# RikVoorhaar/tt-sketch

Hardware: AMD Instinct MI355X
Metric: TT-cores sketched/sec (fp64) + achieved MFMA % for d=6 n=200 r=50 stream_sketch (higher is better)
Workload: dtype f64

## Files before the change

### include/ttsk.h

```cpp
#ifndef TTSK_H
#define TTSK_H

#include <stddef.h>
#include <stdint.h>

#ifdef __cplusplus
extern "C" {
#endif

typedef enum {
    TTSK_OK = 0,
    TTSK_ERR_HIP = -1,
    TTSK_ERR_ARG = -2,
    TTSK_ERR_UNSUPPORTED = -3,
    TTSK_ERR_COMM = -4
} ttsk_status;

#define TTSK_NUM_STREAMS 8

int ttsk_init(int device);
int ttsk_shutdown(void);
const char *ttsk_last_error(void);
int ttsk_device_info(char *name, size_t name_len, int *num_cu, size_t *hbm_bytes);
int ttsk_malloc(void **dev, size_t bytes);
// ... 38 lines not shown
                         double *out, int64_t out_stride, int accumulate, int stream);
int ttsk_tt_sketch_sum(int nb, int d, const int64_t *n, const int64_t *s, const int64_t *lt, const int64_t *l_lo,
                       const int64_t *l_hi, const int64_t *rt, const int64_t *r_lo, const int64_t *r_hi,
                       const double *const *X, const double *const *DL, const double *const *DR,
                       double *out, int accumulate, int stream);
int ttsk_chain_step(int nb, int n, int K1, int A, int A2, int J, const double *const *W, int64_t w_c,
                    const double *const *X, int64_t x_j, int64_t x_k, int64_t x_c, int64_t x_extent,
                    const double *E, double *const *T, double *const *Out, int stream);
int ttsk_chain_step_wide(int nb, int n, int K1, int A, int A2, int J, const double *const *W, int64_t w_c,
                         const double *const *X, int64_t x_j, int64_t x_k, int64_t x_c, int64_t x_extent,
                         const double *E, double *const *T, double *const *Out, int stream);
int ttsk_chain_step_sum(int nb, int n, int K1, int A, int A2, int J, const double *const *W, int64_t w_c,
                        const double *const *X, int64_t x_j, int64_t x_k, int64_t x_c, int64_t x_extent,
                        const double *E, double *T, int64_t t_b, int64_t t_ld, int64_t t_extent,
                        double *const *Out, int stream);
int ttsk_dense_left_pass(const double *X, int64_t n0, int64_t n1, int64_t n2, int64_t C, int64_t n4, int l,
                         const double *A0, const double *A1t, const double *A2t, const double *A3, double *Z0, double *Z1,
                         double *Z2, double *E3, int stream);
int64_t ttsk_tt_sketch_size(int d, const int64_t *n, const int64_t *l_lo, const int64_t *l_hi,
                            const int64_t *r_lo, const int64_t *r_hi);
int ttsk_prof_enable(int on);
int ttsk_mfma_f64_peak_probe(double *tflops);
int ttsk_ndtri_rate_probe(double *gsamples);
int ttsk_prof_read(int cls, int64_t *launches, double *total_ms, double *flops);
int ttsk_prof_kernel_name(int cls, char *buf, size_t len);

int ttsk_hash_u64(uint64_t *host_vals, size_t n);
int ttsk_inds_to_rand_double(const uint64_t *host_idx, const uint64_t *shape, int m, size_t N,
                             int rank_min, int rank_max, uint64_t seed, double *host_out);
int ttsk_inds_to_normal(const int64_t *host_idx, const uint64_t *shape, int m, size_t N,
// ... 131 lines not shown
```

### tt_sketch_amd/_native.py

```python
import ctypes
import os
import re
from ctypes import POINTER, Structure, c_char_p, c_double, c_float, c_int, c_int64, c_size_t, c_uint64, c_void_p
from typing import NamedTuple, Optional

_HERE = os.path.dirname(os.path.abspath(__file__))
LIB_PATH = os.environ.get("TTSK_LIB") or os.path.join(_HERE, "libttsk.so")
HEADER_PATH = os.path.join(os.path.dirname(_HERE), "include", "ttsk.h")

TTSK_ERR_ARG = -2
TTSK_ERR_UNSUPPORTED = -3
NUM_STREAMS = 8


class TtskError(RuntimeError):
    """A HIP / RCCL level failure inside libttsk."""


class TtskUnsupported(TtskError):
    """The fused kernel does not cover this shape (caller composes from ttsk_gemm)."""


class GemmDesc(Structure):
    _fields_ = [(n, c_int64) for n in
# ... 46 lines not shown
    "ttsk_timer_stop": Entry([I, POINTER(c_float)]),
    "ttsk_graph_begin": Entry([I]),
    "ttsk_graph_end": Entry([I, POINTER(P)]),
    "ttsk_graph_launch": Entry([P, I], QUEUE),
    "ttsk_graph_free": Entry([P]),
    "ttsk_gemm": Entry([POINTER(GemmDesc), P, P, P, P, I], QUEUE),
    "ttsk_copy_strided": Entry([P, P, I, POINTER(I64), POINTER(I64), POINTER(I64), I], QUEUE),
    "ttsk_axpby": Entry([P, P, c_double, c_double, S, I], QUEUE),
    "ttsk_sum_slices": Entry([P, P, I, S, S, I, I], QUEUE),
    "ttsk_tt_sketch": Entry([I] + [POINTER(I64)] * 8 + [POINTER(P)] * 3 + [P, I, I], FORK_NEXT),
    "ttsk_tt_sketch_batch": Entry([I, I] + [POINTER(I64)] * 8 + [POINTER(P)] * 3 + [P, I64, I, I], FORK_NEXT),
    "ttsk_tt_sketch_sum": Entry([I, I] + [POINTER(I64)] * 8 + [POINTER(P)] * 3 + [P, I, I], FORK_NEXT),
    "ttsk_chain_step": Entry(_CHAIN + [POINTER(P), POINTER(P), I], QUEUE),
    "ttsk_chain_step_wide": Entry(_CHAIN + [POINTER(P), POINTER(P), I], QUEUE),
    "ttsk_chain_step_sum": Entry(_CHAIN + [P, I64, I64, I64, POINTER(P), I], QUEUE),
    "ttsk_dense_left_pass": Entry([P, I64, I64, I64, I64, I64, I, P, P, P, P, P, P, P, P, I], QUEUE),
    "ttsk_tt_sketch_size": Entry([I] + [POINTER(I64)] * 5, restype=I64),
    "ttsk_prof_enable": Entry([I]),
    "ttsk_mfma_f64_peak_probe": Entry([POINTER(c_double)]),
    "ttsk_ndtri_rate_probe": Entry([POINTER(c_double)]),
    "ttsk_prof_read": Entry([I, POINTER(I64), POINTER(c_double), POINTER(c_double)]),
    "ttsk_prof_kernel_name": Entry([I, c_char_p, S]),
    "ttsk_hash_u64": Entry([P, S]),
    "ttsk_inds_to_rand_double": Entry([P, P, I, S, I, I, U64, P]),
    "ttsk_inds_to_normal": Entry([P, P, I, S, I, I, U64, P]),
    "ttsk_inds_to_sparse_sign": Entry([P, P, I, S, I, I, I, I, U64, P]),
    "ttsk_sparse_normal_dev": Entry([P, I64, POINTER(I), POINTER(U64), I, S, I, I, U64, P, I], QUEUE),
    "ttsk_sparse_normal_table": Entry([POINTER(U64), I, I, I, U64, P, I], QUEUE),
    "ttsk_sparse_sign_dev": Entry([P, I64, POINTER(I), POINTER(U64), I, S, I, I, I, I, U64, P, I], QUEUE),
    "ttsk_sparse_sign_table": Entry([POINTER(U64), I, I, I, I, I, U64, P, I], QUEUE),
# ... 159 lines not shown
```

### tt_sketch_amd/csrc/chain_fused.h

```cpp
#pragma once
#include "chain_plan.h"
#include "skinny.h"

namespace ttsk {

#ifdef TTSK_LAB
#define CF_DIAG(bit) (a.diag & (bit))
#define CF_STAMP(i) do { if (a.stamps && blockIdx.x == 0 && lane == 0 && k - k_beg < 8) a.stamps[((k - k_beg) * CD_WAVES + w) * 8 + (i)] = __builtin_amdgcn_s_memtime(); } while (0)
#else
#define CF_DIAG(bit) 0
#define CF_STAMP(i) do { } while (0)
#endif
#define CF_BARRIER() do { if (!CF_DIAG(4)) lds_barrier(); } while (0)

template <int NQF, int STRQ, int NNF, int STRN, int D, bool WT, int EBUF, int UNR, int KIND, int APC = 0>
__device__ __forceinline__ void cf_piece(const ChainStep &a, const double *Wl, const double *El, int tile, int q0, int prob,
                                         int g, int k_beg, int k_end, int KB1, int w, int lane)
{
    const int x16 = lane & 15, kq = lane >> 4;
    const int AP = APC ? APC : a.AP, A2P = a.A2P;
    const int j0 = 16 * tile;
    const bool jok = j0 + x16 < a.J;
    const uint32_t xlane = !CF_DIAG(1) ? (uint32_t)(((int64_t)(j0 + x16) * a.x_j + (int64_t)kq * a.x_c) * 8) : OOB_OFF;
    const __amdgpu_buffer_rsrc_t rx = make_rsrc(uniform_ptr(a.X[prob]), a.x_extent * 8);
// ... 5 lines not shown
    double ring[D];
#pragma unroll
    for (int d = 0; d < D; ++d) ring[d] = xload((uint32_t)k_beg * kstep + (uint32_t)d * xstep);

    v4d acc2[NNF ? NNF : 1];
    double acc2s[STRN ? STRN : 1];
#pragma unroll
    for (int p = 0; p < NNF; ++p)
#pragma unroll
        for (int t = 0; t < 4; ++t) acc2[p][t] = 0.0;
#pragma unroll
    for (int q = 0; q < STRN; ++q) acc2s[q] = 0.0;

    const int wl_lane = (kq >> 1) * 2 * AP + 2 * (16 * q0 + x16) + (kq & 1);
    const int ws_lane = (kq >> 1) * 2 * AP + 2 * (16 * (q0 + NQF) + (x16 & 3)) + (kq & 1);
    const int el_lane = (kq >> 1) * 2 * A2P + 4 * (x16 >> 1) + 2 * (kq & 1) + (x16 & 1);
    const int es_col = 16 * NNF + (x16 & 3);
    const int es_lane = (kq >> 1) * 2 * A2P + 2 * (kq & 1);

    __amdgpu_buffer_rsrc_t rt;
    if constexpr (WT) rt = make_rsrc(uniform_ptr(a.T[prob]), a.t_extent * 8);

    for (int k = k_beg; k < k_end; ++k) {
        v4d acc1[NQF ? NQF : 1];
        double acc1s[STRQ ? STRQ : 1];
#pragma unroll
        for (int p = 0; p < NQF; ++p)
#pragma unroll
            for (int t = 0; t < 4; ++t) acc1[p][t] = 0.0;
#pragma unroll
        for (int q = 0; q < STRQ; ++q) acc1s[q] = 0.0;

        CF_STAMP(0);
// ... 37 lines not shown
            for (int p = 0; p < NQF; ++p)
#pragma unroll
                for (int t = 0; t < 4; ++t)
                    st8(rt, (jok && a0 + 16 * p + 4 * t + kq < a.A) ? tl + (uint32_t)((16 * p + 4 * t) * nJ * 8) : OOB_OFF, acc1[p][t]);
#pragma unroll
            for (int q = 0; q < STRQ; ++q)
                st8(rt, (jok && a0 + 16 * NQF + 4 * q + kq < a.A) ? tl + (uint32_t)((16 * NQF + 4 * q) * nJ * 8) : OOB_OFF, acc1s[q]);
        }
        CF_STAMP(1);
        CF_BARRIER();
        CF_STAMP(2);

        {
            const double *eb = El + (EBUF == 2 ? (k & 1) * a.eunits * 2 : 0) + q0 * 16 * A2P;
            double bf[NNF ? NNF : 1], bs[STRN ? STRN : 1];
            int el0 = el_lane, es0 = es_lane + 4 * (es_col >> 1) + (es_col & 1);
            asm volatile("" : "+v"(el0), "+v"(es0));
            auto efetch = [&](int kap, double (&f)[NNF ? NNF : 1], double (&g)[STRN ? STRN : 1]) {
#pragma unroll
                for (int nn = 0; nn < NNF; ++nn) f[nn] = LDS_UNPAIRED(eb[el0 + kap * 4 * A2P + 32 * nn]);
#pragma unroll
                for (int q = 0; q < STRN; ++q) g[q] = eb[es0 + kap * 4 * A2P + 8 * q];
            };
            double bf2[NNF ? NNF : 1], bs2[STRN ? STRN : 1];
            efetch(0, bf, bs);
            constexpr int KB2C = 4 * NQF + STRQ;
#pragma unroll
            for (int kap = 0; kap < KB2C; ++kap) {
                const int p = kap >> 2, t = kap & 3;
                const double af2 = p < NQF ? acc1[p < NQF ? p : 0][t] : acc1s[t < STRQ ? t : 0];
                if (kap & 1) {
// ... 62 lines not shown
    const __amdgpu_buffer_rsrc_t rx = make_rsrc(uniform_ptr(a.X[prob]), a.x_extent * 8);
    const uint32_t xstep = __builtin_amdgcn_readfirstlane((uint32_t)(4 * a.x_c * 8));
    const uint32_t kstep = __builtin_amdgcn_readfirstlane((uint32_t)(a.x_k * 8));
    const int ITER = KB1 / UNR;
    auto xload = [&](uint32_t so) -> double { return ld8(rx, xlane, __builtin_amdgcn_readfirstlane(so)); };
    double ring[D];
#pragma unroll
    for (int d = 0; d < D; ++d) ring[d] = xload((uint32_t)k_beg * kstep + (uint32_t)d * xstep);

    double acc2[NC];
#pragma unroll
    for (int c = 0; c < NC; ++c) acc2[c] = 0.0;

    const int wl_lane = (kq >> 1) * 2 * AP + 2 * x16 + (kq & 1);
    const int ws_lane = (kq >> 1) * 2 * AP + 2 * (16 * NQF + n4) + (kq & 1);
    const int el_lane = (2 * beta + (kq >> 1)) * 2 * A2P + 4 * (n4 >> 1) + 2 * (kq & 1) + (n4 & 1);
    const int es_lane = (kq >> 1) * 2 * A2P + 4 * (n4 >> 1) + 2 * (kq & 1) + (n4 & 1);

    __amdgpu_buffer_rsrc_t rt;
    if constexpr (WT) rt = make_rsrc(uniform_ptr(a.T[prob]), a.t_extent * 8);

    for (int k = k_beg; k < k_end; ++k) {
        double acc1[NQF], acc1s[STRQ ? STRQ : 1];
#pragma unroll
        for (int p = 0; p < NQF; ++p) acc1[p] = 0.0;
#pragma unroll
        for (int q = 0; q < STRQ; ++q) acc1s[q] = 0.0;
        CF_STAMP(0);
        uint32_t so = (uint32_t)k * kstep + (uint32_t)D * xstep;
        for (int it = 0; it < ITER; ++it) {
            const double *wrun = Wl + it * UNR * 4 * AP;
            const bool last = it == ITER - 1;
// ... 96 lines not shown
                const int c = e / AP, col = e - c * AP;
                if (e < total) Wl[(c >> 1) * 2 * AP + 2 * col + (c & 1)] = v[u];
            }
        }
    }

    unsigned pc = 0;
    int li = 0, nl = 1;
    if constexpr (NWV != 8) {
        pc = a.piece[__builtin_amdgcn_readfirstlane(w)];
        li = __builtin_amdgcn_readfirstlane((pc >> 8) & 255);
        nl = a.nload;
    }
    if (NWV == 8 ? w == 7 : __builtin_amdgcn_readfirstlane(pc >> 16) == CD_NONE) {
        if constexpr (NWV != 8) __builtin_amdgcn_s_setprio(3);
        const int NI = CF_DIAG(2) ? 0 : a.eunits >> 6;
        const uint32_t inv = (uint32_t)(((1ull << 32) + (uint32_t)A2P - 1) / (uint32_t)A2P);
        const int64_t rowstride = (int64_t)a.n * a.A2;
        const int ebuf = a.eunits * 2;
        auto fill = [&](int k) {
            const double *Ek = a.E + (int64_t)k * a.A2;
            double *dst = El + (EBUF == 2 ? (k & 1) * ebuf : 0);
#pragma unroll 2
            for (int m = li; m < NI; m += nl) {
                const uint32_t U = 64u * (uint32_t)m + (uint32_t)lane;
                const uint32_t sec = (uint32_t)(((uint64_t)U * inv) >> 32), u = U - sec * (uint32_t)A2P;
                int row = (int)(2 * sec + (u & 1));
                row = row < a.A ? row : a.A - 1;
                int col = (int)(2 * (u >> 1));
                col = col + 1 < a.A2 ? col : 0;
                __builtin_amdgcn_global_load_lds((const __attribute__((address_space(1))) void *)(Ek + row * rowstride + col),
                                                 (__attribute__((address_space(3))) void *)(dst + m * 128), 16, 0, 0);
            }
        };
        __syncthreads();
        if constexpr (EBUF == 2) {
            if (k_beg < k_end) fill(k_beg);
            for (int k = k_beg; k < k_end; ++k) {
                asm volatile("s_waitcnt vmcnt(0)" ::: "memory");
                CF_STAMP(1);
                CF_BARRIER();
                CF_STAMP(2);
                if (k + 1 < k_end) fill(k + 1);
                CF_STAMP(3);
                CF_BARRIER();
                CF_STAMP(4);
            }
        } else {
// ... 19 lines not shown
        const int kind = __builtin_amdgcn_readfirstlane(pc >> 16), tile = __builtin_amdgcn_readfirstlane(pc & 255);
        constexpr int H = cd_cut(NQF), APC = 16 * NQF + 4 * STRQ;
        if (kind == CD_WHOLE)
            cf_piece<NQF, STRQ, NNF, STRN, D, WT, EBUF, UNR, CD_WHOLE, APC>(a, Wl, El, tile, 0, prob, g, k_beg, k_end, KB1, w, lane);
        else if (kind == CD_FIRST)
            cf_piece<H, 0, NNF, STRN, D, WT, EBUF, UNR, CD_FIRST, APC>(a, Wl, El, tile, 0, prob, g, k_beg, k_end, KB1, w, lane);
        else if (kind == CD_REST)
            cf_piece<NQF - H, STRQ, NNF, STRN, D, WT, EBUF, UNR, CD_REST, APC>(a, Wl, El, tile, H, prob, g, k_beg, k_end, KB1, w, lane);
        else if (kind == CD_ROWS4)
            cf_rows4<NQF, STRQ, NNF, STRN, D, WT, EBUF, UNR, APC>(a, Wl, El, tile, prob, g, k_beg, k_end, KB1, w, lane);
    }
}

int chain_fused_try(const ChainStepArgs &c, int stream, hipStream_t st, bool force = false);

}
```

### tt_sketch_amd/csrc/chain_fused.hip

```cpp
#include <cstdlib>
#include "chain_fused.h"
#include "prof.h"

namespace ttsk {

int launch_chain_step_a(const ChainStep &a, int nf, int str, bool wt, int ebuf, int unr, int waves, size_t lds, int grid, hipStream_t st);
int launch_chain_step_b(const ChainStep &a, int nf, int str, bool wt, int ebuf, int unr, int waves, size_t lds, int grid, hipStream_t st);
int launch_chain_step_c(const ChainStep &a, int nf, int str, bool wt, int ebuf, int unr, int waves, size_t lds, int grid, hipStream_t st);
int launch_chain_step_d(const ChainStep &a, int nf, int str, bool wt, int ebuf, int unr, int waves, size_t lds, int grid, hipStream_t st);
int launch_chain_step_e(const ChainStep &a, int nf, int str, bool wt, int ebuf, int unr, int waves, size_t lds, int grid, hipStream_t st);

static int launch_chain_step(const ChainStep &a, int nf, int str, bool wt, int ebuf, int unr, int waves, size_t lds, int grid, hipStream_t st)
{
    if (nf <= 2) return launch_chain_step_a(a, nf, str, wt, ebuf, unr, waves, lds, grid, st);
    if (nf <= 4) return launch_chain_step_b(a, nf, str, wt, ebuf, unr, waves, lds, grid, st);
    if (nf == 5) return launch_chain_step_c(a, nf, str, wt, ebuf, unr, waves, lds, grid, st);
    if (nf == 6) return launch_chain_step_d(a, nf, str, wt, ebuf, unr, waves, lds, grid, st);
    return launch_chain_step_e(a, nf, str, wt, ebuf, unr, waves, lds, grid, st);
}

int chain_fused_try(const ChainStepArgs &c, int stream, hipStream_t st, bool force)
{
    const int n_cu = device_num_cu();
    if (n_cu < 1) return TTSK_ERR_HIP;
    ChainFusedPlan p;
    if (!chain_fused_plan(c, n_cu, force, p)) return 0;
    ChainStep &a = p.a;
    a.slab = (double *)scratch(stream, SCRATCH_GEMM, (size_t)p.l.slab * 8 + 64);
    if (!a.slab) return TTSK_ERR_HIP;
    ProfBracket prof(st, PROF_CURRENT, p.l.flops,
                     "chain_step_kernel<%d, %d, %d, %d, 5, %s, 1, %d, %d>", p.nq, p.sq, p.nq, p.sq, p.wt ? "true" : "false", p.ebuf, p.unr);
#ifdef TTSK_LAB
    { static int dg = [] { const char *e = getenv("TTSK_CF_DIAG"); return e ? atoi(e) : 0; }(); a.diag = dg; }
    static int stamps_on = [] { const char *e = getenv("TTSK_CF_STAMPS"); return e ? atoi(e) : 0; }();
#else
    constexpr int stamps_on = 0;
#endif
    long long *stamps_dev = nullptr;
    if (stamps_on) {
        if (hipMalloc(&stamps_dev, 8 * CD_WAVES * 8 * 8) != hipSuccess) return TTSK_ERR_HIP;
        (void)hipMemset(stamps_dev, 0, 8 * CD_WAVES * 8 * 8);
        a.stamps = stamps_dev;
    }
    int rc = launch_chain_step(a, p.nq, p.sq, p.wt, p.ebuf, p.unr, p.waves, p.l.lds, p.l.grid, st);
    if (stamps_on) {
        long long h[8 * CD_WAVES * 8];
        (void)hipStreamSynchronize(st);
        (void)hipMemcpy(h, stamps_dev, sizeof(h), hipMemcpyDeviceToHost);
        (void)hipFree(stamps_dev);
        long long t0 = 0;
        for (int i = 0; i < 8 * CD_WAVES * 8; ++i) if (h[i] && (!t0 || h[i] < t0)) t0 = h[i];
        fprintf(stderr, "[cf stamps] workgroup 0: cycles since its first stamp; per slice, wave: start | endA | afterB1 | endB | afterB2\n");
        for (int sl = 0; sl < 4; ++sl)
            for (int w = 0; w < CD_WAVES; ++w) {
                const long long *r = h + (sl * CD_WAVES + w) * 8;
                if (!r[1] && !r[4]) continue;
                fprintf(stderr, "  slice %d wave %d: %8lld %8lld %8lld %8lld %8lld\n", sl, w, r[0] ? r[0] - t0 : -1, r[1] - t0, r[2] - t0,
                        r[3] - t0, r[4] - t0);
            }
    }
    if (rc == TTSK_OK) {
        ReduceOut ro{};
        for (int b = 0; b < c.nb; ++b) ro.C[b] = c.Out[b];
        rc = launch_r_reduce(st, a.slab, p.l.red_chunks, p.l.red_m, p.l.red_n, 1, (int64_t)c.J, ro, c.nb, (int64_t)c.A2, (int64_t)1, 1.0, 0);
    }
    return rc == TTSK_OK ? 1 : (rc == 1 ? 0 : rc);
}

// ... 20 lines not shown
```

### tt_sketch_amd/csrc/chain_plan.h

```cpp
#pragma once
#include <algorithm>
#include <cstddef>
#include <cstdint>
#include <cstring>
#include <map>
#include <mutex>
#include <vector>
#include "chain_deal.h"
#include "plan_common.h"

namespace ttsk {

struct ChainStepArgs {
    int nb, n, K1, A, A2, J;
    const double *const *W;
    int64_t w_c;
    const double *const *X;
    int64_t x_j, x_k, x_c, x_extent;
    const double *E;
    double *const *T;
    double *const *Out;
};

struct ChainSumArgs {
    ChainStepArgs s;
    double *Tint;
    int64_t t_b, t_ld, t_extent;
};

struct ChainStep {
    const double *W[SK_MAXB];
    const double *X[SK_MAXB];
    double *T[SK_MAXB];
    const double *E;
    double *slab;
    int nb, wpp, n;
    int K1, A, A2, J;
    int64_t w_c;
    int64_t x_j, x_k, x_c;
    int64_t x_extent, t_extent;
    int AP, A2P;
    int ebase;
    int eunits;
    int xcd_map;
    unsigned int piece[CD_WAVES];
    int nload;
    int diag;
    long long *stamps;
};

constexpr int CF_MAX_DMA = 160;

struct ChainWide {
    const double *W[SK_MAXB];
    const double *X[SK_MAXB];
    double *T[SK_MAXB];
    const double *E;
    double *slab;
    int nb, wpp, nac, n;
    int K1, A, A2, J;
    int64_t w_c;
    int64_t x_j, x_k, x_c;
    int64_t x_extent, t_extent;
    int ac;
    int A2P;
    int ebase;
// ... 90 lines not shown
    int na_run;
    bool wt;
    ChainLaunch l;
};

inline void chain_tile_split(int r, int &nf, int &str)
{
    const int rem = r % 16;
    nf = r / 16;
    if (rem == 0) str = 0;
    else if (rem <= 4) str = 1;
    else if (rem <= 8) str = 2;
    else { nf += 1; str = 0; }
}

inline void chain_phase_a_runs(int K1, int &unr, int &KB1)
{
    const int kb = (K1 + 3) / 4;
    const int pad25 = (kb + 24) / 25 * 25, pad5 = (kb + 4) / 5 * 5;
    unr = pad25 <= pad5 + 1 ? 25 : 5;
    KB1 = unr == 25 ? pad25 : pad5;
}

inline int chain_fused_plan(const ChainStepArgs &c, int n_cu, bool force, ChainFusedPlan &p)
{
    if (c.nb < 1 || c.nb > SK_MAXB) return 0;
    if (c.J < 1 || c.J > 112 || c.K1 < 1 || c.K1 > 128 || c.A < 4 || c.A2 < 4 || c.n < 1) return 0;
    if ((c.A2 & 1) || ((uintptr_t)c.E & 15)) return 0;
    int nq, sq, nn, sn;
    chain_tile_split(c.A, nq, sq);
    chain_tile_split(c.A2, nn, sn);
    if (nq != nn || sq != sn || nq + (sq ? 1 : 0) > 7 || nq < 1) return 0;
    if (c.x_j < 0 || c.x_k < 0 || c.x_c < 0 || c.w_c < c.A) return 0;
    p = ChainFusedPlan{};
    ChainStep &a = p.a;
    a.nb = c.nb; a.n = c.n; a.K1 = c.K1; a.A = c.A; a.A2 = c.A2; a.J = c.J;
    a.w_c = c.w_c; a.x_j = c.x_j; a.x_k = c.x_k; a.x_c = c.x_c; a.x_extent = c.x_extent;
    a.E = c.E;
    int unr, KB1;
    chain_phase_a_runs(c.K1, unr, KB1);
    const int KB2 = nq * 4 + sq;
    if (!force && 2 * c.K1 < c.A) return 0;
    a.AP = 16 * nq + 4 * sq;
    a.A2P = c.A2;
    if (a.AP < 4 * KB2) return 0;
    const int64_t wl = (int64_t)4 * KB1 * a.AP;
    a.ebase = (int)((wl + 1) & ~(int64_t)1);
    const int64_t units = (int64_t)2 * KB2 * a.A2P;
    a.eunits = (int)cdiv(units, 64) * 64;
    if (a.eunits / 64 > CF_MAX_DMA) return 0;
    const int ebuf = nq <= 4 ? 2 : 1;
    const size_t lds = ((size_t)a.ebase + (size_t)a.eunits * 2 * ebuf) * 8;
    if (lds > 160 * 1024) return 0;
    if ((c.x_extent + c.x_k + 132 * c.x_c) * 8 >= (1ll << 32) - 64) return 0;
    if ((int64_t)c.A * c.n * c.A2 * 8 >= (1ll << 32) - 64) return 0;
    const bool wt = c.T != nullptr;
    a.t_extent = (int64_t)c.A * c.n * c.J;
    if (wt && (a.t_extent + (int64_t)16 * c.n * c.J) * 8 >= (1ll << 32) - 64) return 0;
    const int cus = n_cu;
    int wpp = cus / c.nb > 0 ? cus / c.nb : 1;
    if (wpp > c.n) wpp = c.n;
    a.wpp = wpp;
    const ChainDeal deal = chain_deal(c.J, c.A, c.A2, nq, sq, nn, sn, KB1, c.n >= 2 * wpp);
    if (deal.waves == CD_WAVES) {
        bool taken[CD_WAVES] = {};
// ... 367 lines not shown
```

### tt_sketch_amd/csrc/common.h

```cpp
#pragma once
#include <hip/hip_runtime.h>
#include <cstdarg>
#include <cstdint>
#include <cstdio>
#include <utility>
#include "plan_common.h"
#include "ttsk.h"
#include "wave.h"

namespace ttsk {

void set_error(const char *fmt, ...);
hipStream_t stream_of(int s);
int ensure_init();
int device_num_cu();
enum { SCRATCH_DRIVER = 0, SCRATCH_GEMM = 1, SCRATCH_MISC = 2, SCRATCH_ORTH = 3, SCRATCH_SLOTS = 4 };
void *scratch(int stream, int slot, size_t bytes);
enum { PA_PINV_HOST = 0, PA_PINV_DEV, PA_DEFERRED, PA_PINV_BATCH_VD, PA_DEFERRED_PINNED, PA_SLOTS };
void *persistent_alloc(int key, size_t bytes, bool host, bool zero);

#define TTSK_HIP(call)                                                          \
    do {                                                                        \
        hipError_t e_ = (call);                                                 \
        if (e_ != hipSuccess) {                                                 \
            ttsk::set_error("%s failed: %s (%s:%d)", #call, hipGetErrorString(e_), \
                            __FILE__, __LINE__);                                \
            return TTSK_ERR_HIP;                                                \
        }                                                                       \
    } while (0)

#define TTSK_ARG(cond, ...)                                                     \
    do {                                                                        \
        if (!(cond)) {                                                          \
            ttsk::set_error(__VA_ARGS__);                                       \
// ... 60 lines not shown
```

### tt_sketch_amd/csrc/runtime.hip

```cpp
#include <atomic>
#include <cstring>
#include <mutex>
#include "common.h"

namespace ttsk {

static thread_local char g_err[512] = "";
static hipStream_t g_streams[TTSK_NUM_STREAMS];
static hipEvent_t g_ev_start[TTSK_NUM_STREAMS], g_ev_stop[TTSK_NUM_STREAMS];
static hipEvent_t g_ev_sync[TTSK_NUM_STREAMS];
static bool g_init = false;
static int g_device = -1;
static std::mutex g_mu;

void set_error(const char *fmt, ...)
{
    va_list ap;
    va_start(ap, fmt);
    vsnprintf(g_err, sizeof(g_err), fmt, ap);
    va_end(ap);
}

int ensure_init()
{
// ... 128 lines not shown
    for (int i = 0; i < TTSK_NUM_STREAMS; ++i) {
        TTSK_HIP(hipStreamCreateWithFlags(&g_streams[i], hipStreamNonBlocking));
        TTSK_HIP(hipEventCreate(&g_ev_start[i]));
        TTSK_HIP(hipEventCreate(&g_ev_stop[i]));
        TTSK_HIP(hipEventCreateWithFlags(&g_ev_sync[i], hipEventDisableTiming));
    }
    g_device = device;
    g_init = true;
    return TTSK_OK;
}

int ttsk_shutdown(void)
{
    std::lock_guard<std::mutex> lk(g_mu);
    if (!g_init) return TTSK_OK;
    for (int i = 0; i < TTSK_NUM_STREAMS; ++i) {
        (void)hipStreamSynchronize(g_streams[i]);
        (void)hipStreamDestroy(g_streams[i]);
        (void)hipEventDestroy(g_ev_start[i]);
        (void)hipEventDestroy(g_ev_stop[i]);
        (void)hipEventDestroy(g_ev_sync[i]);
        for (int k = 0; k < SCRATCH_SLOTS; ++k) {
            if (g_scratch[i][k]) (void)hipFree(g_scratch[i][k]);
            g_scratch[i][k] = nullptr;
            g_scratch_bytes[i][k] = 0;
        }
    }
    for (int k = 0; k < PA_SLOTS; ++k) {
        if (g_pa[k]) (void)(g_pa_host[k] ? hipHostFree(g_pa[k]) : hipFree(g_pa[k]));
        g_pa[k] = nullptr;
    }
    for (auto &k : g_lds_raised) k.store(nullptr, std::memory_order_relaxed);
// ... 149 lines not shown
```

### tt_sketch_amd/csrc/tt_fused.hip

```cpp
#include <algorithm>
#include <cstdlib>
#include <vector>
#include "common.h"
#include "prof.h"
#include "skinny.h"
#include "chain_fused.h"
#include "chain_wide.h"
#include "chain_sum.h"
#include "tt_chain.h"
#include "stream_small.h"

namespace ttsk {

static int gemm(int cls, const ttsk_gemm_desc &d, const double *A, const double *B, double *C, int stream)
{
    ProfClass pc(cls);
    return ttsk_gemm(&d, A, B, C, nullptr, stream);
}

struct BatchPtrs {
    const double *A[SK_MAXB], *B[SK_MAXB];
    double *C[SK_MAXB];
};

// ... 201 lines not shown
    const bool merged = nb > 1 && mu < d - 1 && c.packedL(mu);
    if (merged) {
        c.t_inter[mu] = 1;
        const int64_t ldt = (int64_t)nb * sp;
        double *T0 = c.Tp0(0, mu);
        for (int b = 0; b < nb; ++b) { p.A[b] = c.Lp(b, mu - 1); p.B[b] = c.Xc(b, mu); p.C[b] = T0 + (size_t)b * sp; }
        ttsk_gemm_desc g1 = gemm_desc2(lfull, sp, 1, sn, 1, 0, lfull, 0, nn * sp, 1, nn * ldt, 1, 0);
        g1.batch = nn; g1.b_b = sp; g1.c_b = ldt;
        CK(gemm_batch(2, nb, g1, p, c.aux, c.st_aux));
        BatchPtrs q{};
        q.A[0] = T0; q.B[0] = c.DL[mu]; q.C[0] = c.Lp(0, mu);
        CK(gemm_batch(3, 1, gemm_desc2((int64_t)nb * sp, lt[mu + 1], lfull, nn, 1, nn * ldt, ldt, nn * lt[mu + 1], lt[mu + 1], 1,
                                  lt[mu + 1], 1, 0), q, c.aux, c.st_aux));
        return TTSK_OK;
    }
    for (int b = 0; b < nb; ++b) { p.A[b] = c.Lp(b, mu - 1); p.B[b] = c.Xc(b, mu); p.C[b] = c.Tp0(b, mu); }
    CK(gemm_batch(mu == d - 1 ? 5 : 2, nb, gemm_desc2(lfull, nn * sp, 1, sn, 1, 0, lfull, 0, nn * sp, 1, nn * sp, 1, 0), p,
                  c.aux, c.st_aux));
    if (mu < d - 1) {
        BatchPtrs q{};
        for (int b = 0; b < nb; ++b) { q.A[b] = c.Tp0(b, mu); q.B[b] = c.DL[mu]; q.C[b] = c.Lp(b, mu); }
        CK(gemm_batch(3, nb, gemm_desc2(sp, lt[mu + 1], 1, lfull * nn, 1, 0, sp, 0, lt[mu + 1], 1, lt[mu + 1], 1, 0), q,
                      c.aux, c.st_aux));
    }
    return TTSK_OK;
}

static int run_chains(Ctx &c, bool left)
{
    const char *single = getenv("TTSK_SINGLE_STREAM");
// ... 42 lines not shown
static int psi_omega(const Ctx &c, int mu, int q, bool do_psi, bool do_omega)
{
    const int nb = c.nb, d = c.d;
    const int64_t sp = c.s[mu + 1], nn = c.n[mu];
    hipStream_t stq = stream_of(q);
    const int jr = d - 2 - mu;
    const int64_t ldr = mu < d - 1 ? c.rt[jr + 1] : 0, r = mu < d - 1 ? c.rw(jr) : 1;
    int rc = 0;
    BatchPtrs p{};
    if (!do_psi) {
    } else if (mu == 0) {
        for (int b = 0; b < nb; ++b) { p.A[b] = c.Xc(b, 0); p.B[b] = c.Rslice(b, jr); p.C[b] = c.sum ? c.P0(b) : c.outb(b) + c.psi_at[0]; }
        CK(gemm_batch(5, nb, gemm_desc2(nn, r, 1, sp, sp, 0, 1, 0, ldr, 1, r, 1, c.sum ? 0 : c.accumulate), p, q, stq));
        if (c.sum) CK(ttsk_sum_slices(c.out + c.psi_at[0], c.P0(0), nb, c.szP0, (size_t)(nn * r), c.accumulate, q));
    } else if (mu == d - 1) {
        const size_t len = (size_t)(c.lw(mu - 1) * nn);
        if (c.sum)
            CK(ttsk_sum_slices(c.out + c.psi_at[mu], c.Tslice(0, mu), nb, c.szT[mu], len, c.accumulate, q));
        else
            for (int b = 0; b < nb; ++b) {
                if (c.accumulate) CK(ttsk_axpby(c.outb(b) + c.psi_at[mu], c.Tslice(b, mu), 1.0, 1.0, len, q));
                else TTSK_HIP(hipMemcpyAsync(c.outb(b) + c.psi_at[mu], c.Tslice(b, mu), len * 8, hipMemcpyDeviceToDevice, stq));
            }
    } else if (c.sum && sp <= sum_psi_split) {
        CK(psi_sum_one_product(c, mu, q));
    } else {
        const int64_t l = c.lw(mu - 1), ldt = c.t_ld(mu);
        if (c.sum && !c.t_inter[mu]) {
            const StreamSmallSumArgs sa{nb, 0 , (int)sp, (int)r, c.Tslice(0, mu), ldt, (int64_t)c.szT[mu],
                                        c.Rslice(0, jr), ldr, (int64_t)c.szR[jr], c.out + c.psi_at[mu], r, c.accumulate};
            CK(psi_stream(stream_small_sum_try, sa, l * nn, q, stq));
        }
        if (rc == 0) {
            double *blk0 = c.Ps(mu & 1);
            for (int b = 0; b < nb; ++b) {
                p.A[b] = c.Tslice(b, mu); p.B[b] = c.Rslice(b, jr); p.C[b] = c.sum ? blk0 + (size_t)b * c.szPs : c.outb(b) + c.psi_at[mu];
            }
            const int acc = c.sum ? 0 : c.accumulate;
// ... 232 lines not shown
```

### tt_sketch_amd/drm/tensor_train_drm.py

```python
from __future__ import annotations

from typing import List, Optional, Tuple, Union

import numpy as np

from .. import _native as nat
from ..device import DevArray, as_dev, contract
from ..drm_base import CanSlice, handle_transpose
from ..sketching_methods.abstract_methods import (CansketchCP, CansketchDense, CansketchHadamardProduct,
                                                  CansketchOperatorProduct, CansketchSparse, CansketchTT, CanSketchTucker)
from ..utils import random_normal_dev_many


class TensorTrainDRM(CansketchSparse, CansketchTT, CansketchCP, CanSlice, CansketchDense,
                     CanSketchTucker, CansketchOperatorProduct, CansketchHadamardProduct):
    cores: list

    def __init__(self, rank: Union[Tuple[int, ...], int], shape: Tuple[int, ...], transpose: bool,
                 seed: Optional[int] = None, **kwargs) -> None:
        super().__init__(rank, shape, transpose, seed=seed, **kwargs)
        if "cores" in kwargs:
            self.cores = kwargs["cores"]
        else:
            walk = self.shape[::-1] if transpose else self.shape
            rk = (1,) + tuple(self.true_rank)
            k = len(walk) - 1
            self.cores = random_normal_dev_many([(rk[mu], walk[mu], rk[mu + 1]) for mu in range(k)],
                                                [(self.seed << 20) + mu for mu in range(k)],
                                                [1.0 / np.sqrt(rk[mu]) for mu in range(k)])
        self._dev: List[DevArray] = []
        self._dev_src: list = []

    def dev_cores(self) -> List[DevArray]:
        for k, c in enumerate(self.cores):
            if k < len(self._dev) and self._dev_src[k] is c:
                continue
            d = as_dev(c)
            if k < len(self._dev):
                self._dev[k], self._dev_src[k] = d, c
            else:
                self._dev.append(d)
                self._dev_src.append(c)
        return self._dev

    def _core(self, mu) -> DevArray:
        return self.dev_cores()[mu]
# ... 95 lines not shown
```

### tt_sketch_amd/tt_fused.py

```python
from __future__ import annotations

import math
from typing import List, Optional, Tuple

import numpy as np

from . import _native as nat
from .device import DevArray, c_strides
from .drm.tensor_train_drm import TensorTrainDRM
from .paths import SketchMethod, drm_pair
from .tensor import TensorSum, TensorTrain

MAX_BATCH = 32


class TTSketchPlan:

    def __init__(self, shape, tt_rank, left_drm: TensorTrainDRM, right_drm: TensorTrainDRM):
        d = len(shape)
        self.d = d
        self.shape = tuple(int(x) for x in shape)
        self.tt_rank = tuple(int(x) for x in tt_rank)
        arr = nat.i64_array
        self.n = arr(self.shape)
        self.s = arr((1,) + self.tt_rank + (1,))
        self.lt = arr((1,) + tuple(left_drm.true_rank))
        self.rt = arr((1,) + tuple(right_drm.true_rank))
        self.l_lo, self.l_hi = arr(left_drm.rank_min), arr(left_drm.rank_max)
        self.r_lo, self.r_hi = arr(right_drm.rank_min), arr(right_drm.rank_max)
        self._keep = (left_drm.dev_cores(), right_drm.dev_cores())
        for k, c in enumerate(self._keep[0]):
            want = (self.lt[k], self.shape[k], self.lt[k + 1])
            if tuple(c.shape) != want:
                raise ValueError(f"left DRM core {k} has shape {c.shape}, expected {want}")
        for k, c in enumerate(self._keep[1]):
            want = (self.rt[k], self.shape[d - 1 - k], self.rt[k + 1])
            if tuple(c.shape) != want:
                raise ValueError(f"right DRM core {k} has shape {c.shape}, expected {want}")
        self.DL = nat.ptr_array([c.contiguous() for c in self._keep[0]])
        self.DR = nat.ptr_array([c.contiguous() for c in self._keep[1]])
        self.left_rank = tuple(left_drm.rank)
        self.right_rank = tuple(right_drm.rank[::-1])
        self.size = int(nat.lib().ttsk_tt_sketch_size(d, self.n, self.l_lo, self.l_hi, self.r_lo, self.r_hi))
        self._layout = None

    def new_buffer(self) -> DevArray:
        return DevArray.empty((self.size,))

    def core_pointers(self, tt: TensorTrain):
        cores = tt.dev_cores()
        if tuple(tt.shape) != self.shape or tuple(tt.rank) != self.tt_rank:
            raise ValueError(f"TT of shape {tt.shape} / rank {tt.rank} does not fit the plan")
        keep = [c.contiguous() for c in cores]
        return nat.ptr_array(keep), keep

    def run(self, X_ptrs, out: DevArray, accumulate: bool = False, stream: int = 0):
        nat.call("ttsk_tt_sketch", self.d, self.n, self.s, self.lt, self.l_lo, self.l_hi, self.rt,
                 self.r_lo, self.r_hi, X_ptrs, self.DL, self.DR, out, 1 if accumulate else 0, stream)

    def run_batch(self, X_ptrs, nb: int, out: DevArray, out_stride: int, accumulate: bool = False, stream: int = 0):
        nat.call("ttsk_tt_sketch_batch", nb, self.d, self.n, self.s, self.lt, self.l_lo, self.l_hi, self.rt,
                 self.r_lo, self.r_hi, X_ptrs, self.DL, self.DR, out, out_stride,
                 1 if accumulate else 0, stream)

    def run_sum(self, X_ptrs, nb: int, out: DevArray, accumulate: bool = False, stream: int = 0):
        nat.call("ttsk_tt_sketch_sum", nb, self.d, self.n, self.s, self.lt, self.l_lo, self.l_hi, self.rt,
                 self.r_lo, self.r_hi, X_ptrs, self.DL, self.DR, out, 1 if accumulate else 0, stream)

    def views(self, out: DevArray) -> Tuple[List[DevArray], List[DevArray]]:
        d = self.d
        if self._layout is None:
            lr, rr = (1,) + self.left_rank, self.right_rank + (1,)
            shapes = [(lr[mu], self.shape[mu], rr[mu]) for mu in range(d)] + \
                     [(self.left_rank[mu], self.right_rank[mu]) for mu in range(d - 1)]
            off, lay = 0, []
            for shp in shapes:
                lay.append((off, shp, c_strides(shp)))
                off += math.prod(shp)
            self._layout = lay
        if out.strides != (1,):
            out = out.contiguous()
        arrs = [DevArray(out.buf, out.offset + off, shp, st) for off, shp, st in self._layout]
# ... 95 lines not shown
```

Before: 58110.

## Pre-pack DRM cores into LDS image layout for fused chain step

Adds a one-time pack kernel that rearranges each TT-DRM core into the exact per-unit image the fused chain step loads into LDS, cached by pointer. The fused kernel then streams contiguous 16-byte units instead of computing a scattered gather with division and clamping per unit. It also writes the last core's GEMM straight into the output instead of going through a temporary and a copy or axpby. Packing adds a device allocation and a synchronous launch on first batch use, and the cache keyed by raw pointer can go stale if memory is reused.

```diff
diff --git a/include/ttsk.h b/include/ttsk.h
--- a/include/ttsk.h
+++ b/include/ttsk.h
@@ -76,6 +76,8 @@
                         const double *const *X, int64_t x_j, int64_t x_k, int64_t x_c, int64_t x_extent,
                         const double *E, double *T, int64_t t_b, int64_t t_ld, int64_t t_extent,
                         double *const *Out, int stream);
+int ttsk_drm_pack(const double *core, int A, int n, int A2, int stream);
+int ttsk_drm_unpack(const double *core);
 int ttsk_dense_left_pass(const double *X, int64_t n0, int64_t n1, int64_t n2, int64_t C, int64_t n4, int l,
                          const double *A0, const double *A1t, const double *A2t, const double *A3, double *Z0, double *Z1,
                          double *Z2, double *E3, int stream);
diff --git a/tt_sketch_amd/_native.py b/tt_sketch_amd/_native.py
--- a/tt_sketch_amd/_native.py
+++ b/tt_sketch_amd/_native.py
@@ -84,6 +84,8 @@
     "ttsk_chain_step": Entry(_CHAIN + [POINTER(P), POINTER(P), I], QUEUE),
     "ttsk_chain_step_wide": Entry(_CHAIN + [POINTER(P), POINTER(P), I], QUEUE),
     "ttsk_chain_step_sum": Entry(_CHAIN + [P, I64, I64, I64, POINTER(P), I], QUEUE),
+    "ttsk_drm_pack": Entry([P, I, I, I, I], DRAIN_LAST),
+    "ttsk_drm_unpack": Entry([P]),
     "ttsk_dense_left_pass": Entry([P, I64, I64, I64, I64, I64, I, P, P, P, P, P, P, P, P, I], QUEUE),
     "ttsk_tt_sketch_size": Entry([I] + [POINTER(I64)] * 5, restype=I64),
     "ttsk_prof_enable": Entry([I]),
diff --git a/tt_sketch_amd/csrc/chain_fused.h b/tt_sketch_amd/csrc/chain_fused.h
--- a/tt_sketch_amd/csrc/chain_fused.h
+++ b/tt_sketch_amd/csrc/chain_fused.h
@@ -43,9 +43,9 @@
 
     const int wl_lane = (kq >> 1) * 2 * AP + 2 * (16 * q0 + x16) + (kq & 1);
     const int ws_lane = (kq >> 1) * 2 * AP + 2 * (16 * (q0 + NQF) + (x16 & 3)) + (kq & 1);
-    const int el_lane = (kq >> 1) * 2 * A2P + 4 * (x16 >> 1) + 2 * (kq & 1) + (x16 & 1);
+    const int el_lane = e_frag_lane(x16, kq, A2P);
     const int es_col = 16 * NNF + (x16 & 3);
-    const int es_lane = (kq >> 1) * 2 * A2P + 2 * (kq & 1);
+    const int es_lane = e_strip_lane(kq, A2P);
 
     __amdgpu_buffer_rsrc_t rt;
     if constexpr (WT) rt = make_rsrc(uniform_ptr(a.T[prob]), a.t_extent * 8);
@@ -113,7 +113,7 @@
         {
             const double *eb = El + (EBUF == 2 ? (k & 1) * a.eunits * 2 : 0) + q0 * 16 * A2P;
             double bf[NNF ? NNF : 1], bs[STRN ? STRN : 1];
-            int el0 = el_lane, es0 = es_lane + 4 * (es_col >> 1) + (es_col & 1);
+            int el0 = el_lane, es0 = es_lane + e_image_at(0, es_col, A2P);
             asm volatile("" : "+v"(el0), "+v"(es0));
             auto efetch = [&](int kap, double (&f)[NNF ? NNF : 1], double (&g)[STRN ? STRN : 1]) {
 #pragma unroll
@@ -206,8 +206,8 @@
 
     const int wl_lane = (kq >> 1) * 2 * AP + 2 * x16 + (kq & 1);
     const int ws_lane = (kq >> 1) * 2 * AP + 2 * (16 * NQF + n4) + (kq & 1);
-    const int el_lane = (2 * beta + (kq >> 1)) * 2 * A2P + 4 * (n4 >> 1) + 2 * (kq & 1) + (n4 & 1);
-    const int es_lane = (kq >> 1) * 2 * A2P + 4 * (n4 >> 1) + 2 * (kq & 1) + (n4 & 1);
+    const int el_lane = e_image_at(4 * beta + kq, n4, A2P);
+    const int es_lane = e_image_at(kq, n4, A2P);
 
     __amdgpu_buffer_rsrc_t rt;
     if constexpr (WT) rt = make_rsrc(uniform_ptr(a.T[prob]), a.t_extent * 8);
@@ -334,24 +334,39 @@
     }
     if (NWV == 8 ? w == 7 : __builtin_amdgcn_readfirstlane(pc >> 16) == CD_NONE) {
         if constexpr (NWV != 8) __builtin_amdgcn_s_setprio(3);
+#ifdef TTSK_LAB
+        if (CF_DIAG(8)) {
+            if (li > 0) { __syncthreads(); return; }
+            nl = 1;
+        }
+#endif
         const int NI = CF_DIAG(2) ? 0 : a.eunits >> 6;
-        const uint32_t inv = (uint32_t)(((1ull << 32) + (uint32_t)A2P - 1) / (uint32_t)A2P);
+        const uint32_t inv = e_image_inv(A2P);
         const int64_t rowstride = (int64_t)a.n * a.A2;
         const int ebuf = a.eunits * 2;
-        auto fill = [&](int k) {
+        auto fill_gather = [&](int k) {
             const double *Ek = a.E + (int64_t)k * a.A2;
             double *dst = El + (EBUF == 2 ? (k & 1) * ebuf : 0);
 #pragma unroll 2
             for (int m = li; m < NI; m += nl) {
-                const uint32_t U = 64u * (uint32_t)m + (uint32_t)lane;
-                const uint32_t sec = (uint32_t)(((uint64_t)U * inv) >> 32), u = U - sec * (uint32_t)A2P;
-                int row = (int)(2 * sec + (u & 1));
-                row = row < a.A ? row : a.A - 1;
-                int col = (int)(2 * (u >> 1));
-                col = col + 1 < a.A2 ? col : 0;
-                __builtin_amdgcn_global_load_lds((const __attribute__((address_space(1))) void *)(Ek + row * rowstride + col),
+                const EUnit un = e_image_unit(64u * (uint32_t)m + (uint32_t)lane, inv, a.A, a.A2, A2P);
+                __builtin_amdgcn_global_load_lds((const __attribute__((address_space(1))) void *)(Ek + un.row * rowstride + un.col),
                                                  (__attribute__((address_space(3))) void *)(dst + m * 128), 16, 0, 0);
             }
+        };
+        const uint32_t lane16 = 16u * (uint32_t)lane;
+        auto fill_packed = [&](int k) {
+            const char *src = (const char *)(a.Epk + ((int64_t)k * a.eunits + 64 * li) * 2);
+            double *dst = El + (EBUF == 2 ? (k & 1) * ebuf : 0);
+#pragma unroll 2
+            for (int m = li; m < NI; m += nl, src += 1024 * nl)
+                __builtin_amdgcn_global_load_lds((const __attribute__((address_space(1))) void *)(src + lane16),
+                                                 (__attribute__((address_space(3))) void *)(dst + m * 128), 16, 0, 0);
+        };
+        const bool packed = a.Epk != nullptr;
+        auto fill = [&](int k) {
+            if (packed) fill_packed(k);
+            else fill_gather(k);
         };
         __syncthreads();
         if constexpr (EBUF == 2) {
@@ -401,4 +416,6 @@
 
 int chain_fused_try(const ChainStepArgs &c, int stream, hipStream_t st, bool force = false);
 
+const double *drm_packed_lookup(const double *E, int A, int n, int A2, int A2P, int eunits);
+
 }
diff --git a/tt_sketch_amd/csrc/chain_fused.hip b/tt_sketch_amd/csrc/chain_fused.hip
--- a/tt_sketch_amd/csrc/chain_fused.hip
+++ b/tt_sketch_amd/csrc/chain_fused.hip
@@ -28,6 +28,7 @@
     ChainStep &a = p.a;
     a.slab = (double *)scratch(stream, SCRATCH_GEMM, (size_t)p.l.slab * 8 + 64);
     if (!a.slab) return TTSK_ERR_HIP;
+    a.Epk = drm_packed_lookup(c.E, c.A, c.n, c.A2, a.A2P, a.eunits);
     ProfBracket prof(st, PROF_CURRENT, p.l.flops,
                      "chain_step_kernel<%d, %d, %d, %d, 5, %s, 1, %d, %d>", p.nq, p.sq, p.nq, p.sq, p.wt ? "true" : "false", p.ebuf, p.unr);
 #ifdef TTSK_LAB
@@ -51,7 +52,7 @@
         long long t0 = 0;
         for (int i = 0; i < 8 * CD_WAVES * 8; ++i) if (h[i] && (!t0 || h[i] < t0)) t0 = h[i];
         fprintf(stderr, "[cf stamps] workgroup 0: cycles since its first stamp; per slice, wave: start | endA | afterB1 | endB | afterB2\n");
-        for (int sl = 0; sl < 4; ++sl)
+        for (int sl = 0; sl < 8; ++sl)
             for (int w = 0; w < CD_WAVES; ++w) {
                 const long long *r = h + (sl * CD_WAVES + w) * 8;
                 if (!r[1] && !r[4]) continue;
diff --git a/tt_sketch_amd/csrc/chain_pack.hip b/tt_sketch_amd/csrc/chain_pack.hip
--- /dev/null
+++ b/tt_sketch_amd/csrc/chain_pack.hip
@@ -0,0 +1,84 @@
+#include <map>
+#include <mutex>
+#include "chain_fused.h"
+
+namespace ttsk {
+
+struct PackedCore {
+    int A, n, A2, A2P, eunits;
+    double *img;
+};
+
+static std::mutex g_pack_mu;
+static std::map<const double *, PackedCore> g_packed;
+
+__global__ __launch_bounds__(256) void chain_pack_kernel(const double *__restrict__ E, double *__restrict__ Epk, int A, int n, int A2, int A2P,
+                                                         int eunits, uint32_t inv)
+{
+    const int k = blockIdx.y;
+    const int U = blockIdx.x * 256 + threadIdx.x;
+    if (U >= eunits) return;
+    const EUnit un = e_image_unit((uint32_t)U, inv, A, A2, A2P);
+    const double2 v = *(const double2 *)(E + ((int64_t)un.row * n + k) * A2 + un.col);
+    *(double2 *)(Epk + ((int64_t)k * eunits + U) * 2) = v;
+}
+
+const double *drm_packed_lookup(const double *E, int A, int n, int A2, int A2P, int eunits)
+{
+    std::lock_guard<std::mutex> lk(g_pack_mu);
+    const auto it = g_packed.find(E);
+    if (it == g_packed.end()) return nullptr;
+    const PackedCore &p = it->second;
+    return p.A == A && p.n == n && p.A2 == A2 && p.A2P == A2P && p.eunits == eunits ? p.img : nullptr;
+}
+
+void drm_packed_clear()
+{
+    std::lock_guard<std::mutex> lk(g_pack_mu);
+    for (auto &kv : g_packed) (void)hipFree(kv.second.img);
+    g_packed.clear();
+}
+
+}
+
+using namespace ttsk;
+
+extern "C" int ttsk_drm_pack(const double *core, int A, int n, int A2, int stream)
+{
+    TTSK_STREAM(st, stream);
+    TTSK_ARG(core && A >= 1 && n >= 1 && A2 >= 1, "ttsk_drm_pack: bad argument");
+    int A2P, eunits;
+    if (((uintptr_t)core & 15) || !chain_e_image(A, A2, A2P, eunits) || eunits >= (1 << 16) || n > 65535) {
+        set_error("ttsk_drm_pack: the fused chain step has no image for a core of ranks (%d, %d), n = %d", A, A2, n);
+        return TTSK_ERR_UNSUPPORTED;
+    }
+    if (drm_packed_lookup(core, A, n, A2, A2P, eunits)) return TTSK_OK;
+    int rc = ttsk_drm_unpack(core);
+    if (rc != TTSK_OK) return rc;
+    double *img = nullptr;
+    TTSK_HIP(hipMalloc(&img, (size_t)e_pack_bytes(n, eunits)));
+    rc = launch(chain_pack_kernel, dim3((eunits + 255) / 256, n), 256, 0, st, core, img, A, n, A2, A2P, eunits, e_image_inv(A2P));
+    const hipError_t e = rc == TTSK_OK ? hipStreamSynchronize(st) : hipSuccess;
+    if (rc != TTSK_OK || e != hipSuccess) {
+        (void)hipFree(img);
+        if (rc == TTSK_OK) set_error("ttsk_drm_pack: %s", hipGetErrorString(e));
+        return TTSK_ERR_HIP;
+    }
+    std::lock_guard<std::mutex> lk(g_pack_mu);
+    g_packed[core] = PackedCore{A, n, A2, A2P, eunits, img};
+    return TTSK_OK;
+}
+
+extern "C" int ttsk_drm_unpack(const double *core)
+{
+    double *img = nullptr;
+    {
+        std::lock_guard<std::mutex> lk(g_pack_mu);
+        const auto it = g_packed.find(core);
+        if (it == g_packed.end()) return TTSK_OK;
+        img = it->second.img;
+        g_packed.erase(it);
+    }
+    TTSK_HIP(hipFree(img));
+    return TTSK_OK;
+}
diff --git a/tt_sketch_amd/csrc/chain_plan.h b/tt_sketch_amd/csrc/chain_plan.h
--- a/tt_sketch_amd/csrc/chain_plan.h
+++ b/tt_sketch_amd/csrc/chain_plan.h
@@ -33,6 +33,7 @@
     const double *X[SK_MAXB];
     double *T[SK_MAXB];
     const double *E;
+    const double *Epk;
     double *slab;
     int nb, wpp, n;
     int K1, A, A2, J;
@@ -50,6 +51,26 @@
 };
 
 constexpr int CF_MAX_DMA = 160;
+
+struct EUnit { int row, col; };
+
+constexpr uint32_t e_image_inv(int A2P) { return (uint32_t)(((1ull << 32) + (uint32_t)A2P - 1) / (uint32_t)A2P); }
+
+constexpr EUnit e_image_unit(uint32_t U, uint32_t inv, int A, int A2, int A2P)
+{
+    const uint32_t sec = (uint32_t)(((uint64_t)U * inv) >> 32), u = U - sec * (uint32_t)A2P;
+    int row = (int)(2 * sec + (u & 1));
+    row = row < A ? row : A - 1;
+    int col = (int)(2 * (u >> 1));
+    col = col + 1 < A2 ? col : 0;
+    return EUnit{row, col};
+}
+
+constexpr int e_image_at(int a, int a2, int A2P) { return (a >> 1) * 2 * A2P + 4 * (a2 >> 1) + 2 * (a & 1) + (a2 & 1); }
+constexpr int e_frag_lane(int x16, int kq, int A2P) { return (kq >> 1) * 2 * A2P + 4 * (x16 >> 1) + 2 * (kq & 1) + (x16 & 1); }
+constexpr int e_strip_lane(int kq, int A2P) { return (kq >> 1) * 2 * A2P + 2 * (kq & 1); }
+
+constexpr int64_t e_pack_bytes(int n, int eunits) { return (int64_t)n * eunits * 16; }
 
 struct ChainWide {
     const double *W[SK_MAXB];
@@ -170,6 +191,16 @@
     else { nf += 1; str = 0; }
 }
 
+inline bool chain_e_image(int A, int A2, int &A2P, int &eunits)
+{
+    if (A < 4 || A2 < 4 || (A2 & 1)) return false;
+    int nq, sq;
+    chain_tile_split(A, nq, sq);
+    A2P = A2;
+    eunits = (int)cdiv((int64_t)2 * (nq * 4 + sq) * A2P, 64) * 64;
+    return eunits / 64 <= CF_MAX_DMA;
+}
+
 inline void chain_phase_a_runs(int K1, int &unr, int &KB1)
 {
     const int kb = (K1 + 3) / 4;
@@ -198,13 +229,10 @@
     const int KB2 = nq * 4 + sq;
     if (!force && 2 * c.K1 < c.A) return 0;
     a.AP = 16 * nq + 4 * sq;
-    a.A2P = c.A2;
     if (a.AP < 4 * KB2) return 0;
     const int64_t wl = (int64_t)4 * KB1 * a.AP;
     a.ebase = (int)((wl + 1) & ~(int64_t)1);
-    const int64_t units = (int64_t)2 * KB2 * a.A2P;
-    a.eunits = (int)cdiv(units, 64) * 64;
-    if (a.eunits / 64 > CF_MAX_DMA) return 0;
+    if (!chain_e_image(c.A, c.A2, a.A2P, a.eunits)) return 0;
     const int ebuf = nq <= 4 ? 2 : 1;
     const size_t lds = ((size_t)a.ebase + (size_t)a.eunits * 2 * ebuf) * 8;
     if (lds > 160 * 1024) return 0;
diff --git a/tt_sketch_amd/csrc/common.h b/tt_sketch_amd/csrc/common.h
--- a/tt_sketch_amd/csrc/common.h
+++ b/tt_sketch_amd/csrc/common.h
@@ -18,6 +18,7 @@
 void *scratch(int stream, int slot, size_t bytes);
 enum { PA_PINV_HOST = 0, PA_PINV_DEV, PA_DEFERRED, PA_PINV_BATCH_VD, PA_DEFERRED_PINNED, PA_SLOTS };
 void *persistent_alloc(int key, size_t bytes, bool host, bool zero);
+void drm_packed_clear();
 
 #define TTSK_HIP(call)                                                          \
     do {                                                                        \
diff --git a/tt_sketch_amd/csrc/runtime.hip b/tt_sketch_amd/csrc/runtime.hip
--- a/tt_sketch_amd/csrc/runtime.hip
+++ b/tt_sketch_amd/csrc/runtime.hip
@@ -166,8 +166,9 @@
 {
     std::lock_guard<std::mutex> lk(g_mu);
     if (!g_init) return TTSK_OK;
+    for (int i = 0; i < TTSK_NUM_STREAMS; ++i) (void)hipStreamSynchronize(g_streams[i]);
+    drm_packed_clear();
     for (int i = 0; i < TTSK_NUM_STREAMS; ++i) {
-        (void)hipStreamSynchronize(g_streams[i]);
         (void)hipStreamDestroy(g_streams[i]);
         (void)hipEventDestroy(g_ev_start[i]);
         (void)hipEventDestroy(g_ev_stop[i]);
diff --git a/tt_sketch_amd/csrc/tt_fused.hip b/tt_sketch_amd/csrc/tt_fused.hip
--- a/tt_sketch_amd/csrc/tt_fused.hip
+++ b/tt_sketch_amd/csrc/tt_fused.hip
@@ -239,6 +239,13 @@
                                   lt[mu + 1], 1, 0), q, c.aux, c.st_aux));
         return TTSK_OK;
     }
+    if (mu == d - 1 && !c.sum) {
+        if (c.lw(mu - 1) == 0) return TTSK_OK;
+        for (int b = 0; b < nb; ++b) { p.A[b] = c.Lslice(b, mu - 1); p.B[b] = c.Xc(b, mu); p.C[b] = c.outb(b) + c.psi_at[mu]; }
+        CK(gemm_batch(5, nb, gemm_desc2(c.lw(mu - 1), nn * sp, 1, sn, 1, 0, lfull, 0, nn * sp, 1, nn * sp, 1, c.accumulate), p, c.aux,
+                      c.st_aux));
+        return TTSK_OK;
+    }
     for (int b = 0; b < nb; ++b) { p.A[b] = c.Lp(b, mu - 1); p.B[b] = c.Xc(b, mu); p.C[b] = c.Tp0(b, mu); }
     CK(gemm_batch(mu == d - 1 ? 5 : 2, nb, gemm_desc2(lfull, nn * sp, 1, sn, 1, 0, lfull, 0, nn * sp, 1, nn * sp, 1, 0), p,
                   c.aux, c.st_aux));
@@ -311,14 +318,7 @@
         CK(gemm_batch(5, nb, gemm_desc2(nn, r, 1, sp, sp, 0, 1, 0, ldr, 1, r, 1, c.sum ? 0 : c.accumulate), p, q, stq));
         if (c.sum) CK(ttsk_sum_slices(c.out + c.psi_at[0], c.P0(0), nb, c.szP0, (size_t)(nn * r), c.accumulate, q));
     } else if (mu == d - 1) {
-        const size_t len = (size_t)(c.lw(mu - 1) * nn);
-        if (c.sum)
-            CK(ttsk_sum_slices(c.out + c.psi_at[mu], c.Tslice(0, mu), nb, c.szT[mu], len, c.accumulate, q));
-        else
-            for (int b = 0; b < nb; ++b) {
-                if (c.accumulate) CK(ttsk_axpby(c.outb(b) + c.psi_at[mu], c.Tslice(b, mu), 1.0, 1.0, len, q));
-                else TTSK_HIP(hipMemcpyAsync(c.outb(b) + c.psi_at[mu], c.Tslice(b, mu), len * 8, hipMemcpyDeviceToDevice, stq));
-            }
+        if (c.sum) CK(ttsk_sum_slices(c.out + c.psi_at[mu], c.Tslice(0, mu), nb, c.szT[mu], (size_t)(c.lw(mu - 1) * nn), c.accumulate, q));
     } else if (c.sum && sp <= sum_psi_split) {
         CK(psi_sum_one_product(c, mu, q));
     } else {
diff --git a/tt_sketch_amd/drm/tensor_train_drm.py b/tt_sketch_amd/drm/tensor_train_drm.py
--- a/tt_sketch_amd/drm/tensor_train_drm.py
+++ b/tt_sketch_amd/drm/tensor_train_drm.py
@@ -1,5 +1,7 @@
 from __future__ import annotations
 
+import ctypes
+import sys
 from typing import List, Optional, Tuple, Union
 
 import numpy as np
@@ -10,6 +12,35 @@
 from ..sketching_methods.abstract_methods import (CansketchCP, CansketchDense, CansketchHadamardProduct,
                                                   CansketchOperatorProduct, CansketchSparse, CansketchTT, CanSketchTucker)
 from ..utils import random_normal_dev_many
+
+
+class _PackedCores:
+
+    def __init__(self):
+        self.cores: List[DevArray] = []
+
+    def add(self, core: DevArray) -> None:
+        if any(c is core for c in self.cores):
+            return
+        A, n, A2 = (int(x) for x in core.shape)
+        try:
+            nat.call("ttsk_drm_pack", ctypes.c_void_p(core.ptr), A, n, A2, 0)
+        except nat.TtskUnsupported:
+            return
+        self.cores.append(core)
+
+    def release(self) -> None:
+        cores, self.cores = self.cores, []
+        for c in cores:
+            nat.call("ttsk_drm_unpack", ctypes.c_void_p(c.ptr))
+
+    def __del__(self):
+        if sys.is_finalizing():
+            return
+        try:
+            self.release()
+        except Exception:
+            pass
 
 
 class TensorTrainDRM(CansketchSparse, CansketchTT, CansketchCP, CanSlice, CansketchDense,
@@ -30,6 +61,15 @@
                                                 [1.0 / np.sqrt(rk[mu]) for mu in range(k)])
         self._dev: List[DevArray] = []
         self._dev_src: list = []
+        self._packed = _PackedCores()
+
+    def pack_for_chain(self) -> None:
+        for k, c in enumerate(self.dev_cores()):
+            if k >= 1 and c.ndim == 3 and c.is_contiguous():
+                self._packed.add(c)
+
+    def close(self) -> None:
+        self._packed.release()
 
     def dev_cores(self) -> List[DevArray]:
         for k, c in enumerate(self.cores):
diff --git a/tt_sketch_amd/tt_fused.py b/tt_sketch_amd/tt_fused.py
--- a/tt_sketch_amd/tt_fused.py
+++ b/tt_sketch_amd/tt_fused.py
@@ -29,6 +29,7 @@
         self.l_lo, self.l_hi = arr(left_drm.rank_min), arr(left_drm.rank_max)
         self.r_lo, self.r_hi = arr(right_drm.rank_min), arr(right_drm.rank_max)
         self._keep = (left_drm.dev_cores(), right_drm.dev_cores())
+        self._drms = (left_drm, right_drm)
         for k, c in enumerate(self._keep[0]):
             want = (self.lt[k], self.shape[k], self.lt[k + 1])
             if tuple(c.shape) != want:
@@ -59,13 +60,23 @@
                  self.r_lo, self.r_hi, X_ptrs, self.DL, self.DR, out, 1 if accumulate else 0, stream)
 
     def run_batch(self, X_ptrs, nb: int, out: DevArray, out_stride: int, accumulate: bool = False, stream: int = 0):
+        if nb >= 2:
+            self._pack()
         nat.call("ttsk_tt_sketch_batch", nb, self.d, self.n, self.s, self.lt, self.l_lo, self.l_hi, self.rt,
                  self.r_lo, self.r_hi, X_ptrs, self.DL, self.DR, out, out_stride,
                  1 if accumulate else 0, stream)
 
     def run_sum(self, X_ptrs, nb: int, out: DevArray, accumulate: bool = False, stream: int = 0):
+        if nb >= 2:
+            self._pack()
         nat.call("ttsk_tt_sketch_sum", nb, self.d, self.n, self.s, self.lt, self.l_lo, self.l_hi, self.rt,
                  self.r_lo, self.r_hi, X_ptrs, self.DL, self.DR, out, 1 if accumulate else 0, stream)
+
+    def _pack(self):
+        if self._drms is not None:
+            for drm in self._drms:
+                drm.pack_for_chain()
+            self._drms = None
 
     def views(self, out: DevArray) -> Tuple[List[DevArray], List[DevArray]]:
         d = self.d
```

Result: faster. 59270, median of 6 (+2.0%).
